# ALVI-Labs/frankenstein

Measured on AMD Instinct MI355X. Metric: neural frames/sec (train fwd+bwd+AdamW, whole job), higher is better.
Workload: dtype bf16; 1 GPU; brainformer-small (6L d=384 6x64 heads, N=6144 tokens) + 2-block perceiver, L1 head; fwd+bwd+clip+AdamW; per_gpu_batch=32, global_batch=32, frames_T=600, electrodes=256, parallelism=dp1, weights=random-init (seed 42)

## Files before the change

frankenstein_amd/csrc/gemm.hip:

```cpp
#include <type_traits>

#include "fk_common.h"

namespace {

#ifndef FK_EPI_UNROLL
#define FK_EPI_UNROLL 1
#endif
#include "gemm_tile.h"

struct NtArgs {
  const void* A; const void* B; void* C;
  const void* bias; const void* res;
  int64_t lda, ldb, ldc, ldr, res_rows;
  int M, N, K, vec_epi;
  int mode;
  void* aux; int64_t ldaux;
  const float* rope_table; int64_t rope_bs; int rope_T, rope_off, rope_D, rope_cols;
  int rope_qcols; int64_t rope_qoff;
};

#ifndef FK_NT_STORES_GEMM
#define FK_NT_STORES_GEMM 1
#endif
// ... 787 lines not shown
#pragma unroll
          for (int j = 0; j < 2; ++j) mma32<T>(acc[i][j], fb[j], fa[i]);
        __builtin_amdgcn_sched_barrier(0);
        if (s < 2) issue_b(fill_b, s); else issue_a(fill_a, s - 2);
        __builtin_amdgcn_sched_barrier(0);
      }
#else
      issue_b(fill_b, -1);
      issue_a(fill_a, -1);
#endif
      sa = sa == 2 ? 0 : sa + 1;
      sb ^= 1;
    }
    asm volatile("s_barrier" ::: "memory");
    char* stg = wave < 4 ? aslot(sa == 0 ? 2 : sa - 1) + wave * 8192 : bslot(sb ^ 1) + (wave - 4) * 8192;
#ifdef FK_RING_PROBE_NOEPI
    if (acc[0][0][0] == 123.456f) ((float*)p.C)[tid] = acc[MT - 1][1][3];
#else
#pragma unroll
    for (int i = 0; i < MT; ++i) {
      f32x16 (&sub)[1][2] = *reinterpret_cast<f32x16 (*)[1][2]>(&acc[i][0]);
      nt_epilogue<T, TO, true, 1, false, EPI>(p, sub, stg, m0 + wm * WM + i * 32, n0 + wn * 64, lane, false);
    }
#endif
  }
}

constexpr int R192_A = 256 * ROW_BYTES, R192_B = 192 * ROW_BYTES, R192_LDS = 3 * R192_A + 2 * R192_B + 8192;
static_assert(R192_LDS <= 160 * 1024, "LDS of a CU");

template <typename TO, int EPI>
__global__ __launch_bounds__(512, 2) void gemm_nt_ring192_kernel(NtArgs p) {
  using T = bf16_t;
  constexpr int BM_ = 256, BN_ = 192, APW = 4, BPW = 3, NT6 = 6;
  extern __shared__ __attribute__((aligned(16))) char smem[];
  auto aslot = [&](int i) -> char* { return smem + i * R192_A; };
  auto bslot = [&](int i) -> char* { return smem + 3 * R192_A + i * R192_B; };
  const int tid = threadIdx.x, lane = tid & 63;
  const int wave = __builtin_amdgcn_readfirstlane(tid >> 6);
  const int li = lane & 31, lh = lane >> 5;
  const int ntn = p.N / BN_;
  const TileRange tr = tile_range(((p.M + BM_ - 1) / BM_) * ntn);
  const int nbx = tr.nbx, t_end = tr.end;
  const int nk = p.K / 64;

  const T* srcA[APW];
  const T* srcB[BPW];
  auto set_a = [&](int tile) {
    const int m0 = (tile / ntn) * BM_;
#pragma unroll
    for (int j = 0; j < APW; ++j) srcA[j] = dma_src(p.A, m0, p.M, p.lda, wave * APW + j, lane);
  };
  auto set_b = [&](int tile) {
    const int n0 = (tile % ntn) * BN_;
#pragma unroll
    for (int j = 0; j < BPW; ++j) srcB[j] = dma_src<ROW_BYTES, false>(p.B, n0, p.N, p.ldb, wave * BPW + j, lane);
  };
  int atile = tr.beg + tr.jb, akt = 0, btile = atile, bkt = 0;
  if (atile < t_end) { set_a(atile); set_b(btile); }
  auto issue_a = [&](int slot, int part) __attribute__((always_inline)) {
    if (atile >= t_end) return;
    char* as = aslot(slot);
#pragma unroll
    for (int j = 0; j < APW; ++j)
      if (part < 0 || j / 2 == part)
        __builtin_amdgcn_global_load_lds((glb_void_t*)(srcA[j] + akt * 64), (lds_void_t*)(as + (wave * APW + j) * 1024), 16, 0, 0);
    if (part != 0) { if (++akt == nk) { akt = 0; atile += nbx; if (atile < t_end) set_a(atile); } }
  };
  auto issue_b = [&](int slot, int part) __attribute__((always_inline)) {
    if (btile >= t_end) return;
    char* bs = bslot(slot);
#pragma unroll
    for (int j = 0; j < BPW; ++j)
      if (part < 0 || (j + 1) / 2 == part)
        __builtin_amdgcn_global_load_lds((glb_void_t*)(srcB[j] + bkt * 64), (lds_void_t*)(bs + (wave * BPW + j) * 1024), 16, 0, 0);
    if (part != 0) { if (++bkt == nk) { bkt = 0; btile += nbx; if (btile < t_end) set_b(btile); } }
  };
  issue_a(0, -1);
  issue_b(0, -1);
  issue_a(1, -1);
  int sa = 0, sb = 0;
  for (int tile = tr.beg + tr.jb; tile < t_end; tile += nbx) {
    const int m0 = (tile / ntn) * BM_, n0 = (tile % ntn) * BN_;
    const bool last_tile = tile + nbx >= t_end;
    f32x16 acc[NT6];
#pragma unroll
    for (int j = 0; j < NT6; ++j)
#pragma unroll
      for (int r = 0; r < 16; ++r) acc[j][r] = 0.0f;
    for (int kt = 0; kt < nk; ++kt) {
      if (last_tile && kt == nk - 1) vm_wait_barrier<0>(); else vm_wait_barrier<APW>();
      const int fill_a = sa == 0 ? 2 : sa - 1, fill_b = sb ^ 1;
      const char* as = aslot(sa);
      const char* bs = bslot(sb);
#ifndef FK_RING_PROBE_NOMMA
#pragma unroll
      for (int s = 0; s < 4; ++s) {
        Frag<T> fa, fb[NT6];
        nt_frag<T>(fa, as, wave * 32 + li, s, lh);
#pragma unroll
        for (int j = 0; j < NT6; ++j) nt_frag<T>(fb[j], bs, j * 32 + li, s, lh);
#pragma unroll
        for (int j = 0; j < NT6; ++j) mma32<T>(acc[j], fb[j], fa);
        __builtin_amdgcn_sched_barrier(0);
        if (s < 2) issue_b(fill_b, s); else issue_a(fill_a, s - 2);
        __builtin_amdgcn_sched_barrier(0);
      }
#else
      issue_b(fill_b, -1);
      issue_a(fill_a, -1);
#endif
      sa = sa == 2 ? 0 : sa + 1;
      sb ^= 1;
    }
    asm volatile("s_barrier" ::: "memory");
    char* stg = wave < 4 ? aslot(sa == 0 ? 2 : sa - 1) + wave * 8192
              : (wave < 7 ? bslot(sb ^ 1) + (wave - 4) * 8192 : smem + 3 * R192_A + 2 * R192_B);
#ifdef FK_RING_PROBE_NOEPI
    if (acc[0][0] == 123.456f) ((float*)p.C)[tid] = acc[NT6 - 1][3];
#else
#pragma unroll
    for (int c = 0; c < 3; ++c) {
      f32x16 (&sub)[1][2] = *reinterpret_cast<f32x16 (*)[1][2]>(&acc[2 * c]);
      if (EPI == 0 && p.res) nt_epilogue<T, TO, true, 1, true, EPI>(p, sub, stg, m0 + wave * 32, n0 + 64 * c, lane, false);
      else nt_epilogue<T, TO, true, 1, false, EPI>(p, sub, stg, m0 + wave * 32, n0 + 64 * c, lane, false);
    }
#endif
  }
}

static unsigned persistent_grid(int64_t nt) {
  static const int g = [] { const char* e = getenv("FK_NT_GRID_MULT"); const int v = e ? atoi(e) : 4; return v < 1 ? 1 : (v > 64 ? 64 : v); }();
  const int64_t cap = 256LL * g;
  return (unsigned)(nt < cap ? nt : cap);
}

enum NtRoute { NT_RING2, NT_RING192, NT_RING128, NT_BIG, NT_GLDS4, NT_GLDS, NT_STAGED };

template <typename F> static void with_epi(const NtArgs& p, F f) {
  if (p.mode == 1) f(std::integral_constant<int, 1>{});
  else if (p.mode == 2) f(std::integral_constant<int, 2>{});
  else if (p.rope_table) f(std::integral_constant<int, 3>{});
  else f(std::integral_constant<int, 0>{});
}

template <typename TO> static void launch_nt_route(NtRoute route, const NtArgs& p, int64_t M, int64_t N, hipStream_t s) {
  const int64_t nwg = fk_cdiv(M, BM) * fk_cdiv(N, BN);
  const dim3 grid((unsigned)nwg), block(NTHREADS), block8(512);
  auto tiles256 = [&](int bn) { return dim3(persistent_grid(fk_cdiv(M, 256) * fk_cdiv(N, bn))); };
  switch (route) {
    case NT_RING2: {
      static const bool generic = getenv("FK_NT_RING2_GENERIC") != nullptr;
      if (generic) fk_launch_lds<gemm_nt_ring2_kernel<TO, -1>>(tiles256(256), block8, R2_LDS, s, p);
      else with_epi(p, [&](auto epi) { fk_launch_lds<gemm_nt_ring2_kernel<TO, decltype(epi)::value>>(tiles256(256), block8, R2_LDS, s, p); });
      break;
    }
    case NT_RING192: fk_launch_lds<gemm_nt_ring192_kernel<TO, 0>>(tiles256(192), block8, R192_LDS, s, p); break;
    case NT_RING128:
      with_epi(p, [&](auto epi) { fk_launch_lds<gemm_nt_ring_kernel<TO, 128, 128, 3, decltype(epi)::value>>(tiles256(128), block8, Ring<128, 128, 3>::LDS, s, p); });
      break;
    case NT_BIG: fk_launch_lds<gemm_nt_big_kernel<TO, 256>>(tiles256(256), block8, 2 * (256 + 256) * ROW_BYTES, s, p); break;
    case NT_GLDS4: fk_launch_lds<gemm_nt_glds4_kernel<TO>>(grid, block, G4_LDS, s, p); break;
    case NT_GLDS:
      hipLaunchKernelGGL((gemm_nt_glds_kernel<TO>), dim3((unsigned)(nwg < 512 ? nwg : 512)), block, 4 * TILE_BYTES, s, p);
      break;
    case NT_STAGED: hipLaunchKernelGGL((gemm_nt_kernel<bf16_t, TO>), grid, block, 4 * TILE_BYTES, s, p); break;
  }
}

template <typename T> struct TNT;
template <> struct TNT<bf16_t> { static constexpr int BKM = 64, ROWB = 256, CHUNKS = 16, STEPS = 4; };
template <> struct TNT<float> { static constexpr int BKM = 32, ROWB = 512, CHUNKS = 32, STEPS = 2; };

FK_DEV int tn_off_bf16(int row, int bytecol) {
  const int g = bytecol >> 6;
  return row * 256 + (((g ^ (row & 3)) << 6) | (bytecol & 63));
}

template <typename T> FK_DEV void tn_frag(Frag<T>& f, const char* tile, int cb, int s, int lane);
template <> FK_DEV void tn_frag<bf16_t>(Frag<bf16_t>& f, const char* tile, int cb, int s, int lane) {
  const int g = lane >> 4, i = lane & 15, h = g >> 1;
  const int col = cb + 16 * (g & 1) + 4 * (i & 3);
#pragma unroll
  for (int t = 0; t < 2; ++t) {
    const int row = 16 * s + 8 * h + 4 * t + (i >> 2);
    bf16x4 v = lds_read_tr4(reinterpret_cast<const bf16_t*>(tile + tn_off_bf16(row, col * 2)));
#pragma unroll
    for (int e = 0; e < 4; ++e) f.v[4 * t + e] = v[e];
  }
}
template <> FK_DEV void tn_frag<float>(Frag<float>& f, const char* tile, int cb, int s, int lane) {
  const int h = lane >> 5, c = cb + (lane & 31);
#pragma unroll
  for (int e = 0; e < 8; ++e)
    f.v[e] = *reinterpret_cast<const float*>(tile + (16 * s + 8 * h + e) * 512 + c * 4);
}

struct TnArgs {
  const void* A; const void* B; float* C; float* ws;
  int64_t lda, ldb, ldc;
  int M, N1, N2, rows_per_split, nsplit, accumulate;
};

template <typename T>
__global__ __launch_bounds__(NTHREADS, 2) void gemm_tn_kernel(TnArgs p) {
  extern __shared__ __attribute__((aligned(16))) char smem[];
  constexpr int BKM = TNT<T>::BKM, ROWB = TNT<T>::ROWB, CHUNKS = TNT<T>::CHUNKS, STEPS = TNT<T>::STEPS;
  constexpr int VEC = KT<T>::VEC;
  constexpr int LOG_CH = (CHUNKS == 16) ? 4 : 5;
  const int tid = threadIdx.x, lane = tid & 63, wave = tid >> 6;
  const int wm = wave >> 1, wn = wave & 1, li = lane & 31, lh = lane >> 5;
  const int nt2 = (p.N2 + BN - 1) / BN, ntiles = ((p.N1 + BM - 1) / BM) * nt2;
  const unsigned L = xcd_remap(blockIdx.x, gridDim.x);
  const int split = (int)(L / ntiles), tile = (int)(L % ntiles);
  const int a0 = (tile / nt2) * BM, b0 = (tile % nt2) * BN;
  const int mbeg = split * p.rows_per_split;
  const int mend = min(p.M, mbeg + p.rows_per_split);
  const T* A = (const T*)p.A;
  const T* B = (const T*)p.B;

  f32x16 acc[2][2];
#pragma unroll
  for (int i = 0; i < 2; ++i)
#pragma unroll
    for (int j = 0; j < 2; ++j)
#pragma unroll
      for (int r = 0; r < 16; ++r) acc[i][j][r] = 0.0f;

  u32x4 ra[4], rb[4];
  auto gload = [&](int mrow0) {
#pragma unroll
    for (int i = 0; i < 4; ++i) {
      const int id = tid + NTHREADS * i, row = id >> LOG_CH, ch = id & (CHUNKS - 1);
      const int m = mrow0 + row, ca = a0 + ch * VEC, cb = b0 + ch * VEC;
      u32x4 z = {0u, 0u, 0u, 0u};
      ra[i] = (m < mend && ca < p.N1) ? *reinterpret_cast<const u32x4*>(A + (int64_t)m * p.lda + ca) : z;
      rb[i] = (m < mend && cb < p.N2) ? *reinterpret_cast<const u32x4*>(B + (int64_t)m * p.ldb + cb) : z;
    }
  };
  auto lds_off = [&](int row, int ch) -> int {
    if constexpr (sizeof(T) == 2) return tn_off_bf16(row, ch * 16);
    else return row * ROWB + ch * 16;
  };
  auto lstore = [&](int buf) {
    char* as = smem + buf * 2 * TILE_BYTES;
    char* bs = as + TILE_BYTES;
#pragma unroll
    for (int i = 0; i < 4; ++i) {
      const int id = tid + NTHREADS * i, row = id >> LOG_CH, ch = id & (CHUNKS - 1);
      *reinterpret_cast<u32x4*>(as + lds_off(row, ch)) = ra[i];
      *reinterpret_cast<u32x4*>(bs + lds_off(row, ch)) = rb[i];
    }
  };

  const int nk = (mend - mbeg + BKM - 1) / BKM;
  if (nk > 0) {
    gload(mbeg);
    lstore(0);
  }
  __syncthreads();
  for (int kt = 0; kt < nk; ++kt) {
    if (kt + 1 < nk) gload(mbeg + (kt + 1) * BKM);
    const char* as = smem + (kt & 1) * 2 * TILE_BYTES;
    const char* bs = as + TILE_BYTES;
#pragma unroll
    for (int s = 0; s < STEPS; ++s) {
      Frag<T> fa[2], fb[2];
#pragma unroll
      for (int i = 0; i < 2; ++i) tn_frag<T>(fa[i], as, wm * 64 + i * 32, s, lane);
#pragma unroll
      for (int j = 0; j < 2; ++j) tn_frag<T>(fb[j], bs, wn * 64 + j * 32, s, lane);
#pragma unroll
      for (int i = 0; i < 2; ++i)
#pragma unroll
        for (int j = 0; j < 2; ++j) mma32<T>(acc[i][j], fa[i], fb[j]);
    }
    if (kt + 1 < nk) lstore((kt + 1) & 1);
    __syncthreads();
  }

  float* out = (p.nsplit > 1) ? p.ws + (int64_t)split * p.N1 * p.N2 : p.C;
  const int64_t ldo = (p.nsplit > 1) ? p.N2 : p.ldc;
  const bool accum = (p.nsplit == 1) && p.accumulate;
#pragma unroll
  for (int j = 0; j < 2; ++j) {
    const int n = b0 + wn * 64 + j * 32 + li;
    if (n >= p.N2) continue;
#pragma unroll
    for (int i = 0; i < 2; ++i)
#pragma unroll
      for (int r = 0; r < 16; ++r) {
        const int m = a0 + wm * 64 + i * 32 + acc_row(r, lh);
        if (m >= p.N1) continue;
        float* dst = out + (int64_t)m * ldo + n;
        *dst = accum ? (*dst + acc[i][j][r]) : acc[i][j][r];
      }
  }
}

constexpr int TG_A = 384, TG_B = 128, TG_K = 32;
#ifndef FK_TG_NS
#define FK_TG_NS 4
#endif
constexpr int TG_NS = FK_TG_NS;
constexpr int TG_A_ROW = TG_A * 2, TG_B_ROW = TG_B * 2;
constexpr int TG_A_BYTES = TG_K * TG_A_ROW, TG_B_BYTES = TG_K * TG_B_ROW, TG_STAGE = TG_A_BYTES + TG_B_BYTES;

template <int PITCH> FK_DEV int tg_off(int row, int bytecol) {
  return row * PITCH + (bytecol & ~255) + ((((bytecol >> 6) ^ row) & 3) << 6) + (bytecol & 63);
}
template <int OFF> FK_DEV bf16x4 tr_read(unsigned base) {
  s16x4 r;
  asm volatile("ds_read_b64_tr_b16 %0, %1 offset:%2" : "=v"(r) : "v"(base), "n"(OFF) : "memory");
  return __builtin_bit_cast(bf16x4, r);
}
template <int N> FK_DEV void lgkm_wait() {
  asm volatile("s_waitcnt lgkmcnt(%0)" ::"n"(N) : "memory");
  __builtin_amdgcn_sched_barrier(0);
}
template <int PITCH, int S> FK_DEV void tg_frag(Frag<bf16_t>& f, unsigned base) {
  const bf16x4 v0 = tr_read<(16 * S) * PITCH>(base), v1 = tr_read<(16 * S + 4) * PITCH>(base);
#pragma unroll
  for (int e = 0; e < 4; ++e) { f.v[e] = v0[e]; f.v[4 + e] = v1[e]; }
}
FK_DEV unsigned lds_addr(const char* p) {
  return (unsigned)(__UINTPTR_TYPE__)((__attribute__((address_space(3))) const char*)p);
}

template <int TB>
__global__ __launch_bounds__(512, 2) void gemm_tn_big_kernel(TnArgs p) {
  constexpr int B_ROW = TB == 128 ? 256 : 512, B_BYTES = TG_K * B_ROW, STAGE = TG_A_BYTES + B_BYTES, NJ = TB / 64, WB = TB / 2;
  using T = bf16_t;
  extern __shared__ __attribute__((aligned(16))) char smem[];
  const int tid = threadIdx.x, lane = tid & 63;
  const int wave = __builtin_amdgcn_readfirstlane(tid >> 6);
  const int wm = wave >> 1, wn = wave & 1, li = lane & 31, lh = lane >> 5;
  const int nt2 = p.N2 / TB, ntiles = (p.N1 / TG_A) * nt2;
  const unsigned L = xcd_remap(blockIdx.x, gridDim.x);
  const int split = (int)(L / ntiles), tile = (int)(L % ntiles);
  const int a0 = (tile / nt2) * TG_A, b0 = (tile % nt2) * TB;
  const int mbeg = split * p.rows_per_split;
  const int mend = min(p.M, mbeg + p.rows_per_split);
  const int nk = (mend - mbeg) / TG_K;

  constexpr int APW = TG_A_BYTES / 8192, BPW = B_BYTES / 8192, PER = APW + BPW;
  const T* srcA[APW];
  const T* srcB[BPW];
#pragma unroll
  for (int j = 0; j < APW; ++j) {
    const int o = (wave * APW + j) * 1024 + lane * 16, row = o / TG_A_ROW, bc = o % TG_A_ROW;
    const int sc = (bc & ~255) + ((((bc >> 6) ^ row) & 3) << 6) + (bc & 63);
    srcA[j] = (const T*)p.A + (int64_t)(mbeg + row) * p.lda + a0 + sc / 2;
  }
#pragma unroll
  for (int j = 0; j < BPW; ++j) {
    const int o = (wave * BPW + j) * 1024 + lane * 16, row = o / B_ROW, bc = o % B_ROW;
    int sc = (bc & ~255) + ((((bc >> 6) ^ row) & 3) << 6) + (bc & 63);
    if (sc >= TB * 2) sc = 0;
    srcB[j] = (const T*)p.B + (int64_t)(mbeg + row) * p.ldb + b0 + sc / 2;
  }
  const int64_t astep = (int64_t)TG_K * p.lda, bstep = (int64_t)TG_K * p.ldb;
  auto stage = [&](int buf) {
    char* as = smem + buf * STAGE;
#pragma unroll
    for (int j = 0; j < APW; ++j) {
      __builtin_amdgcn_global_load_lds((glb_void_t*)srcA[j], (lds_void_t*)(as + (wave * APW + j) * 1024), 16, 0, 0);
      srcA[j] += astep;
    }
#pragma unroll
    for (int j = 0; j < BPW; ++j) {
      __builtin_amdgcn_global_load_lds((glb_void_t*)srcB[j], (lds_void_t*)(as + TG_A_BYTES + (wave * BPW + j) * 1024), 16, 0, 0);
      srcB[j] += bstep;
    }
  };

  unsigned fbase[3 + NJ];
  {
    const int g = lane >> 4, i = lane & 15, row = 8 * (g >> 1) + (i >> 2), dc = 16 * (g & 1) + 4 * (i & 3);
#pragma unroll
    for (int q = 0; q < 3; ++q) fbase[q] = lds_addr(smem) + tg_off<TG_A_ROW>(row, (wm * 96 + q * 32 + dc) * 2);
#pragma unroll
    for (int q = 0; q < NJ; ++q) fbase[3 + q] = lds_addr(smem) + TG_A_BYTES + tg_off<B_ROW>(row, (wn * WB + q * 32 + dc) * 2);
  }

  f32x16 acc[3][NJ];
#pragma unroll
  for (int i = 0; i < 3; ++i)
#pragma unroll
    for (int j = 0; j < NJ; ++j)
#pragma unroll
      for (int r = 0; r < 16; ++r) acc[i][j][r] = 0.0f;

#pragma unroll
  for (int s = 0; s < TG_NS - 1; ++s)
    if (s < nk) stage(s);
  int slot = 0;
  for (int kt = 0; kt < nk; ++kt) {
    const int after = nk - 1 - kt;
    if (after >= TG_NS - 2) vm_wait_barrier<(TG_NS - 2) * PER>();
    else if (after == 3) vm_wait_barrier<3 * PER>();
    else if (after == 2) vm_wait_barrier<2 * PER>();
    else if (after == 1) vm_wait_barrier<PER>();
    else vm_wait_barrier<0>();
    if (kt + TG_NS - 1 < nk) stage(slot == 0 ? TG_NS - 1 : slot - 1);
    const unsigned bo = slot * STAGE;
    slot = slot == TG_NS - 1 ? 0 : slot + 1;
    Frag<T> f0[3 + NJ], f1[3 + NJ];
#pragma unroll
    for (int q = 0; q < 3; ++q) tg_frag<TG_A_ROW, 0>(f0[q], fbase[q] + bo);
#pragma unroll
    for (int q = 0; q < NJ; ++q) tg_frag<B_ROW, 0>(f0[3 + q], fbase[3 + q] + bo);
#pragma unroll
    for (int q = 0; q < 3; ++q) tg_frag<TG_A_ROW, 1>(f1[q], fbase[q] + bo);
#pragma unroll
    for (int q = 0; q < NJ; ++q) tg_frag<B_ROW, 1>(f1[3 + q], fbase[3 + q] + bo);
    lgkm_wait<2 * (3 + NJ)>();
#pragma unroll
    for (int i = 0; i < 3; ++i)
#pragma unroll
      for (int j = 0; j < NJ; ++j) mma32<T>(acc[i][j], f0[i], f0[3 + j]);
    lgkm_wait<0>();
#pragma unroll
    for (int i = 0; i < 3; ++i)
#pragma unroll
      for (int j = 0; j < NJ; ++j) mma32<T>(acc[i][j], f1[i], f1[3 + j]);
  }

  float* out = (p.nsplit > 1) ? p.ws + (int64_t)split * p.N1 * p.N2 : p.C;
  const int64_t ldo = (p.nsplit > 1) ? p.N2 : p.ldc;
  const bool accum = (p.nsplit == 1) && p.accumulate;
#pragma unroll
  for (int j = 0; j < NJ; ++j) {
    const int n = b0 + wn * WB + j * 32 + li;
#pragma unroll
    for (int i = 0; i < 3; ++i)
#pragma unroll
      for (int r = 0; r < 16; ++r) {
        const int m = a0 + wm * 96 + i * 32 + acc_row(r, lh);
        float* dst = out + (int64_t)m * ldo + n;
        *dst = accum ? (*dst + acc[i][j][r]) : acc[i][j][r];
      }
  }
}

__global__ __launch_bounds__(256) void reduce_slabs4_kernel(const float* ws, float* C, int64_t ldc, int N1, int N2, int nsplit, int accumulate) {
  const int64_t total = (int64_t)N1 * N2, total4 = total >> 2;
  const int n2v = N2 >> 2;
  for (int64_t i = blockIdx.x * (int64_t)blockDim.x + threadIdx.x; i < total4; i += (int64_t)gridDim.x * blockDim.x) {
    const f32x4* src = reinterpret_cast<const f32x4*>(ws) + i;
    f32x4 s = {0.0f, 0.0f, 0.0f, 0.0f};
    int k = 0;
    for (; k + 8 <= nsplit; k += 8) {
      f32x4 v[8];
#pragma unroll
      for (int u = 0; u < 8; ++u) v[u] = src[(int64_t)(k + u) * total4];
#pragma unroll
      for (int u = 0; u < 8; ++u) s += v[u];
    }
    for (; k < nsplit; ++k) s += src[(int64_t)k * total4];
    f32x4* dst = reinterpret_cast<f32x4*>(C + (i / n2v) * ldc + (i % n2v) * 4);
    if (accumulate) s += *dst;
    *dst = s;
  }
}
__global__ void reduce_slabs_kernel(const float* ws, float* C, int64_t ldc, int N1, int N2, int nsplit, int accumulate) {
  const int64_t total = (int64_t)N1 * N2;
  for (int64_t i = blockIdx.x * (int64_t)blockDim.x + threadIdx.x; i < total; i += (int64_t)gridDim.x * blockDim.x) {
    float s = 0.0f;
    for (int k = 0; k < nsplit; ++k) s += ws[k * total + i];
    float* dst = C + (i / N2) * ldc + (i % N2);
    *dst = accumulate ? (*dst + s) : s;
  }
}

template <typename T>
__global__ __launch_bounds__(256) void colsum_partial_kernel(const T* X, int64_t ld, float* part, int rows, int cols, int rows_per_blk) {
  constexpr int N = 16 / sizeof(T);
  __shared__ float red[256 * N];
  const int r0 = blockIdx.y * rows_per_blk, r1 = min(rows, r0 + rows_per_blk);
  const int cvt = (cols + N - 1) / N;
  {
    const int cv0 = blockIdx.x * 256;
    const int cvn = min(256, cvt - cv0), groups = 256 / cvn;
    const int vec = threadIdx.x % cvn, grp = threadIdx.x / cvn;
    float acc[N];
#pragma unroll
    for (int e = 0; e < N; ++e) acc[e] = 0.0f;
    if (grp < groups) {
      const T* p = X + (int64_t)(cv0 + vec) * N;
      for (int r = r0 + grp; r < r1; r += groups) {
        if constexpr (sizeof(T) == 2) {
          bf16x8 v = *reinterpret_cast<const bf16x8*>(p + (int64_t)r * ld);
#pragma unroll
          for (int e = 0; e < N; ++e) acc[e] += (float)v[e];
        } else {
          f32x4 v = *reinterpret_cast<const f32x4*>(p + (int64_t)r * ld);
#pragma unroll
          for (int e = 0; e < N; ++e) acc[e] += v[e];
        }
      }
    }
    __syncthreads();
#pragma unroll
    for (int e = 0; e < N; ++e) red[threadIdx.x * N + e] = acc[e];
    __syncthreads();
    if (threadIdx.x < cvn) {
#pragma unroll
      for (int e = 0; e < N; ++e) {
        float sm = 0.0f;
        for (int g2 = 0; g2 < groups; ++g2) sm += red[(g2 * cvn + threadIdx.x) * N + e];
        part[(int64_t)blockIdx.y * cols + (cv0 + threadIdx.x) * N + e] = sm;
      }
    }
  }
}
template <typename T>
__global__ void colsum_partial_scalar_kernel(const T* X, int64_t ld, float* part, int rows, int cols, int rows_per_blk) {
  const int c = blockIdx.x * blockDim.x + threadIdx.x;
  if (c >= cols) return;
  const int r0 = blockIdx.y * rows_per_blk, r1 = min(rows, r0 + rows_per_blk);
  float s = 0.0f;
  for (int r = r0; r < r1; ++r) s += to_f32<T>(X[(int64_t)r * ld + c]);
  part[(int64_t)blockIdx.y * cols + c] = s;
}
__global__ __launch_bounds__(256) void colsum_final_kernel(const float* part, float* out, int cols, int nblk, int accumulate) {
  __shared__ float red[256];
  const int c = blockIdx.x * 64 + (threadIdx.x & 63), g = threadIdx.x >> 6;
  float s = 0.0f;
  if (c < cols)
    for (int k = g; k < nblk; k += 4) s += part[(int64_t)k * cols + c];
  red[threadIdx.x] = s;
  __syncthreads();
  if (g == 0 && c < cols) {
    const float t = (red[threadIdx.x] + red[threadIdx.x + 64]) + (red[threadIdx.x + 128] + red[threadIdx.x + 192]);
    out[c] = accumulate ? out[c] + t : t;
  }
}

int tn_splits(int64_t M, int64_t N1, int64_t N2, int bkm) {
  const int64_t tiles = fk_cdiv(N1, BM) * fk_cdiv(N2, BN);
  int64_t want = fk_cdiv(1024, tiles);
  const int64_t maxs = fk_cdiv(M, (int64_t)bkm * 4);
  if (want >= 8) want = (want + 7) / 8 * 8;
  if (want > maxs) want = maxs;
  if (want < 1) want = 1;
  return (int)want;
}
bool tn_big_ok(int64_t M, int64_t N1, int64_t N2, int dtype) {
  return dtype == FK_BF16 && M % TG_K == 0 && M >= 16384 && N1 % TG_A == 0 && (N2 % TG_B == 0 || N2 % 192 == 0);
}
int tn_big_tb(int64_t N1, int64_t N2) {
  static const bool no192 = getenv("FK_TN_NO_192") != nullptr;
  if (N2 % TG_B != 0) return 192;
  return (N2 % 192 == 0 && N1 >= 2048 && !no192) ? 192 : TG_B;
}
int tn_big_splits(int64_t M, int64_t N1, int64_t N2) {
  const int64_t tiles = (N1 / TG_A) * (N2 / tn_big_tb(N1, N2));
  static const int mult = [] { const char* e = getenv("FK_TN_SPLIT_MULT"); const int v = e ? atoi(e) : 1; return v < 1 ? 1 : (v > 8 ? 8 : v); }();
  int64_t want = 256 / tiles * mult;
  const int64_t maxs = M / 512;
  if (want > maxs) want = maxs;
  if (want < 1) want = 1;
  return (int)want;
}
int colsum_blocks(int64_t rows) {
  int64_t b = fk_cdiv(rows, 256);
  if (b > 512) b = 512;
  if (b < 1) b = 1;
  return (int)b;
}

}

bool fk_qkv_rope_fused_ok(int64_t M, int64_t N, int64_t K, int64_t lda, int64_t ldb, int64_t ldc, const void* bias, int64_t T, int64_t D, int64_t rot_cols, int64_t q_cols, int dtype);
int fk_qkv_rope_fused_launch(const void* A, int64_t lda, const void* W, int64_t ldb, void* C, int64_t ldc, int64_t M, int64_t N, const float* table, int64_t table_bs, int64_t T, int64_t pos_off, int64_t rot_cols, int64_t q_cols, int64_t q_off, void* stream);
bool fk_mlp_up_fused_ok(int64_t M, int64_t H, int64_t K, int64_t lda, int64_t ldb, int64_t ldh, int64_t ldg, int dtype);
int fk_mlp_up_fused_launch(const void* A, int64_t lda, const void* W13, int64_t ldb, void* H13, int64_t ldh, void* G, int64_t ldg, int64_t M, int64_t H, void* stream);

extern "C" {

struct RopeSpec { const float* table; int64_t bs; int T, off, D, cols; int qcols; int64_t qoff; };

static int launch_nt(const char* name, const void* A, int64_t lda, const void* B, int64_t ldb, void* C, int64_t ldc, int64_t M,
                     int64_t N, int64_t K, const void* bias, const void* residual, int64_t ldr, int64_t res_rows, int dtype,
                     int out_dtype, int mode, void* aux, int64_t ldaux, void* stream, RopeSpec rope = RopeSpec{nullptr, 0, 1, 0, 2, 0, 0, 0}) {
  FK_CHECK_ARG(dtype == FK_F32 || dtype == FK_BF16, "%s: bad dtype %d", name, dtype);
  FK_CHECK_ARG(out_dtype == dtype || out_dtype == FK_F32, "%s: out_dtype must equal dtype or be f32", name);
  const int vec = dtype == FK_BF16 ? 8 : 4;
  FK_CHECK_ARG(M > 0 && N > 0 && K > 0, "%s: empty problem M=%lld N=%lld K=%lld", name, (long long)M, (long long)N, (long long)K);
  FK_CHECK_ARG(M < (1LL << 31) && N < (1LL << 31) && K < (1LL << 31), "%s: dims must fit int32", name);
  FK_CHECK_ARG(K % vec == 0 && lda % vec == 0 && ldb % vec == 0, "%s: K/lda/ldb must be multiples of %d", name, vec);
  const int64_t ccols = mode == 2 ? 2 * N : N, auxcols = mode == 1 ? N / 2 : (mode == 2 ? 2 * N : 0);
  FK_CHECK_ARG((M == 1 || (lda >= K && ldc >= ccols && ldaux >= auxcols && (!residual || res_rows == 1 || ldr >= N))) && (N == 1 || ldb >= K),
               "%s: leading dimensions must cover their rows (lda=%lld ldb=%lld K=%lld, ldc=%lld for %lld columns, aux %lld for %lld)", name,
               (long long)lda, (long long)ldb, (long long)K, (long long)ldc, (long long)ccols, (long long)ldaux, (long long)auxcols);
  FK_CHECK_ARG(A && B && C, "%s: null pointer", name);
  FK_CHECK_ARG(((uintptr_t)A & 15) == 0 && ((uintptr_t)B & 15) == 0, "%s: A/B must be 16-byte aligned", name);
  const int ovec = 8;
  const bool vec_epi = (N % ovec == 0) && (ldc % ovec == 0) && (((uintptr_t)C & 15) == 0) &&
                       (!residual || (ldr % ovec == 0 && ((uintptr_t)residual & 15) == 0));
  if (mode != 0)
    FK_CHECK_ARG(vec_epi && out_dtype == dtype && aux && ldaux % ovec == 0 && ((uintptr_t)aux & 15) == 0,
                 "%s: fused SwiGLU epilogue needs N %% 8 == 0 and 16-byte aligned, 8-element strided buffers", name);
  if (rope.table)
    FK_CHECK_ARG(vec_epi && rope.D % 8 == 0 && rope.cols % rope.D == 0 && rope.cols <= N && rope.T > 0 && M % rope.T == 0 &&
                 ((uintptr_t)rope.table & 15) == 0, "%s: fused RoPE needs the vector epilogue, D %% 8 == 0 and M %% T == 0", name);
  NtArgs p{A, B, C, bias, residual, lda, ldb, ldc, ldr, res_rows, (int)M, (int)N, (int)K, vec_epi ? 1 : 0, mode, aux, ldaux,
           rope.table, rope.bs, rope.T, rope.off, rope.D, rope.cols, rope.qcols, rope.qoff};
  const int64_t nwg = fk_cdiv(M, BM) * fk_cdiv(N, BN);
  hipStream_t s = (hipStream_t)stream;
  const bool glds = dtype == FK_BF16 && (K % 64 == 0);
  static const bool no_ring = getenv("FK_NT_NO_RING") != nullptr;
  const char* ring_min_env = getenv("FK_NT_RING_MIN_TILES");
  const int ring_min = ring_min_env ? atoi(ring_min_env) : 128;
  const bool wide = glds && M >= 4096 && vec_epi && !no_ring && fk_cdiv(M, 256) * fk_cdiv(N, 256) >= ring_min;
  const NtRoute route = [&] {
    if (wide && (N % 256 == 0 || (N % 128 == 0 && N >= 1024))) return NT_RING2;
    static const bool no_192 = getenv("FK_NT_NO_192") != nullptr;
    if (wide && N % 192 == 0 && N % 256 != 0 && N <= 768 && mode == 0 && !rope.table && !no_192) return NT_RING192;
    if (wide && N % 128 == 0) return NT_RING128;
    if (glds && M >= 4096 && N % 256 == 0 && vec_epi) return NT_BIG;
    static const bool no_g4 = getenv("FK_NT_NO_GLDS4") != nullptr;
    if (glds && nwg <= 256 && !no_g4) return NT_GLDS4;
    return glds ? NT_GLDS : NT_STAGED;
  }();
  if (dtype == FK_F32)
    hipLaunchKernelGGL((gemm_nt_kernel<float, float>), dim3((unsigned)nwg), dim3(NTHREADS), 4 * TILE_BYTES, s, p);
  else if (out_dtype == FK_BF16) launch_nt_route<bf16_t>(route, p, M, N, s);
  else launch_nt_route<float>(route, p, M, N, s);
  FK_CHECK_LAUNCH(name);
  return FK_OK;
}

int fk_gemm_nt(const void* A, int64_t lda, const void* B, int64_t ldb, void* C, int64_t ldc, int64_t M, int64_t N,
               int64_t K, const void* bias, const void* residual, int64_t ldr, int64_t res_rows, int dtype,
               int out_dtype, void* stream) {
  return launch_nt("fk_gemm_nt", A, lda, B, ldb, C, ldc, M, N, K, bias, residual, ldr, res_rows, dtype, out_dtype, 0, nullptr, 0, stream);
}

int fk_gemm_nt_rope(const void* A, int64_t lda, const void* B, int64_t ldb, void* C, int64_t ldc, int64_t M, int64_t N,
                    int64_t K, const void* bias, const float* table, int64_t table_bs, int64_t T, int64_t pos_off, int64_t D,
                    int64_t rot_cols, int64_t q_cols, int64_t q_table_off, int dtype, void* stream) {
  FK_CHECK_ARG(table && T > 0 && D > 0 && rot_cols >= 0, "fk_gemm_nt_rope: bad rope arguments");
  FK_CHECK_ARG(q_cols >= 0 && q_cols <= rot_cols && q_cols % 8 == 0 && q_table_off % 4 == 0, "fk_gemm_nt_rope: bad pre-scaled query table (q_cols %lld, offset %lld)", (long long)q_cols, (long long)q_table_off);
  if (A && B && C && (((uintptr_t)A | (uintptr_t)B | (uintptr_t)C | (uintptr_t)table) & 15) == 0 && M > 0 && pos_off >= 0 &&
      fk_qkv_rope_fused_ok(M, N, K, lda, ldb, ldc, bias, T, D, rot_cols, q_cols, dtype))
    return fk_qkv_rope_fused_launch(A, lda, B, ldb, C, ldc, M, N, table, table_bs, T, pos_off, rot_cols, q_cols, q_table_off, stream);
  return launch_nt("fk_gemm_nt_rope", A, lda, B, ldb, C, ldc, M, N, K, bias, nullptr, 0, 0, dtype, dtype, 0, nullptr, 0, stream,
                   RopeSpec{table, table_bs, (int)T, (int)pos_off, (int)D, (int)rot_cols, (int)q_cols, q_table_off});
}

int fk_gemm_nt_swiglu(const void* A, int64_t lda, const void* W13, int64_t ldb, void* H13, int64_t ldh, void* G,
                      int64_t ldg, int64_t M, int64_t H, int64_t K, int dtype, void* stream) {
  FK_CHECK_ARG(H > 0 && H % 4 == 0, "fk_gemm_nt_swiglu: hidden size must be a multiple of 4");
  if (A && W13 && H13 && G && (((uintptr_t)A | (uintptr_t)W13 | (uintptr_t)H13 | (uintptr_t)G) & 15) == 0 && M > 0 &&
      fk_mlp_up_fused_ok(M, H, K, lda, ldb, ldh, ldg, dtype))
    return fk_mlp_up_fused_launch(A, lda, W13, ldb, H13, ldh, G, ldg, M, H, stream);
  return launch_nt("fk_gemm_nt_swiglu", A, lda, W13, ldb, H13, ldh, M, 2 * H, K, nullptr, nullptr, 0, 0, dtype, dtype, 1, G, ldg, stream);
}

int fk_gemm_nt_dswiglu(const void* dY, int64_t lda, const void* W2T, int64_t ldb, const void* H13, int64_t ldh, void* dH13,
                       int64_t lddh, int64_t M, int64_t H, int64_t K, int dtype, void* stream) {
  FK_CHECK_ARG(H > 0 && H % 8 == 0, "fk_gemm_nt_dswiglu: hidden size must be a multiple of 8");
  FK_CHECK_ARG(lddh % 8 == 0 && ((uintptr_t)dH13 & 15) == 0, "fk_gemm_nt_dswiglu: dH13 must be 16-byte aligned with an 8-element stride");
  return launch_nt("fk_gemm_nt_dswiglu", dY, lda, W2T, ldb, dH13, lddh, M, H, K, nullptr, nullptr, 0, 0, dtype, dtype, 2,
                   const_cast<void*>(H13), ldh, stream);
}

size_t fk_gemm_tn_workspace_bytes(int64_t M, int64_t N1, int64_t N2, int dtype) {
  const int ns = tn_big_ok(M, N1, N2, dtype) ? tn_big_splits(M, N1, N2) : tn_splits(M, N1, N2, dtype == FK_BF16 ? 64 : 32);
  return ns > 1 ? (size_t)ns * N1 * N2 * sizeof(float) : 0;
}

int fk_gemm_tn(const void* A, int64_t lda, const void* B, int64_t ldb, float* C, int64_t ldc, int64_t M, int64_t N1,
               int64_t N2, int accumulate, int dtype, void* workspace, size_t workspace_bytes, void* stream) {
  FK_CHECK_ARG(dtype == FK_F32 || dtype == FK_BF16, "fk_gemm_tn: bad dtype %d", dtype);
  const int vec = dtype == FK_BF16 ? 8 : 4, bkm = dtype == FK_BF16 ? 64 : 32;
  FK_CHECK_ARG(M > 0 && N1 > 0 && N2 > 0, "fk_gemm_tn: empty problem");
  FK_CHECK_ARG(M < (1LL << 31) && N1 < (1LL << 31) && N2 < (1LL << 31), "fk_gemm_tn: dims must fit int32");
  FK_CHECK_ARG(N1 % vec == 0 && N2 % vec == 0 && lda % vec == 0 && ldb % vec == 0,
               "fk_gemm_tn: N1/N2/lda/ldb must be multiples of %d (N1=%lld N2=%lld)", vec, (long long)N1, (long long)N2);
  FK_CHECK_ARG(((uintptr_t)A & 15) == 0 && ((uintptr_t)B & 15) == 0, "fk_gemm_tn: A/B must be 16-byte aligned");
  const bool big = tn_big_ok(M, N1, N2, dtype);
  const int ns = big ? tn_big_splits(M, N1, N2) : tn_splits(M, N1, N2, bkm);
  const size_t need = ns > 1 ? (size_t)ns * N1 * N2 * sizeof(float) : 0;
  FK_CHECK_ARG(workspace_bytes >= need && (need == 0 || workspace), "fk_gemm_tn: workspace too small (%zu < %zu)", workspace_bytes, need);
  int64_t rps = fk_cdiv(fk_cdiv(M, ns), bkm) * bkm;
  TnArgs p{A, B, C, (float*)workspace, lda, ldb, ldc, (int)M, (int)N1, (int)N2, (int)rps, ns, accumulate};
  dim3 grid((unsigned)(fk_cdiv(N1, BM) * fk_cdiv(N2, BN) * ns)), block(NTHREADS);
  hipStream_t s = (hipStream_t)stream;
  if (big) {
    const int tb = tn_big_tb(N1, N2);
    dim3 bgrid((unsigned)((N1 / TG_A) * (N2 / tb) * ns));
    if (tb == 192) {
      constexpr int LDS192 = TG_NS * (TG_A_BYTES + TG_K * 512);
      fk_launch_lds<gemm_tn_big_kernel<192>>(bgrid, dim3(512), LDS192, s, p);
    } else {
      fk_launch_lds<gemm_tn_big_kernel<128>>(bgrid, dim3(512), TG_NS * TG_STAGE, s, p);
    }
  } else if (dtype == FK_BF16) hipLaunchKernelGGL((gemm_tn_kernel<bf16_t>), grid, block, 4 * TILE_BYTES, s, p);
  else hipLaunchKernelGGL((gemm_tn_kernel<float>), grid, block, 4 * TILE_BYTES, s, p);
  FK_CHECK_LAUNCH("fk_gemm_tn");
  if (ns > 1) {
    const int64_t total = N1 * N2;
    if (N2 % 4 == 0 && ldc % 4 == 0 && (((uintptr_t)C | (uintptr_t)workspace) & 15) == 0) {
      int nb = (int)fk_cdiv(total / 4, 256);
      if (nb > 2048) nb = 2048;
      hipLaunchKernelGGL(reduce_slabs4_kernel, dim3(nb), dim3(256), 0, s, (const float*)workspace, C, ldc, (int)N1, (int)N2, ns, accumulate);
    } else {
      int nb = (int)fk_cdiv(total, 256);
      if (nb > 2048) nb = 2048;
      hipLaunchKernelGGL(reduce_slabs_kernel, dim3(nb), dim3(256), 0, s, (const float*)workspace, C, ldc, (int)N1, (int)N2, ns, accumulate);
    }
    FK_CHECK_LAUNCH("fk_gemm_tn(reduce)");
  }
  return FK_OK;
}

size_t fk_colsum_workspace_bytes(int64_t rows, int64_t cols) { return (size_t)colsum_blocks(rows) * cols * sizeof(float); }

int fk_colsum(const void* X, int64_t ld, float* out, int64_t rows, int64_t cols, int accumulate, int dtype,
              void* workspace, size_t workspace_bytes, void* stream) {
  FK_CHECK_ARG(dtype == FK_F32 || dtype == FK_BF16, "fk_colsum: bad dtype %d", dtype);
  FK_CHECK_ARG(rows > 0 && cols > 0 && rows < (1LL << 31) && cols < (1LL << 31), "fk_colsum: bad shape");
  const int nb = colsum_blocks(rows);
  FK_CHECK_ARG(workspace && workspace_bytes >= (size_t)nb * cols * sizeof(float), "fk_colsum: workspace too small");
  const int rpb = (int)fk_cdiv(rows, nb);
  hipStream_t s = (hipStream_t)stream;
  const int vec = dtype == FK_BF16 ? 8 : 4;
  if (cols % vec == 0 && ld % vec == 0 && ((uintptr_t)X & 15) == 0) {
    dim3 grid((unsigned)fk_cdiv(fk_cdiv(cols, vec), 256), (unsigned)nb), block(256);
    if (dtype == FK_BF16) hipLaunchKernelGGL(colsum_partial_kernel<bf16_t>, grid, block, 0, s, (const bf16_t*)X, ld, (float*)workspace, (int)rows, (int)cols, rpb);
    else hipLaunchKernelGGL(colsum_partial_kernel<float>, grid, block, 0, s, (const float*)X, ld, (float*)workspace, (int)rows, (int)cols, rpb);
  } else {
    dim3 grid((unsigned)fk_cdiv(cols, 256), (unsigned)nb), block(256);
    if (dtype == FK_BF16) hipLaunchKernelGGL(colsum_partial_scalar_kernel<bf16_t>, grid, block, 0, s, (const bf16_t*)X, ld, (float*)workspace, (int)rows, (int)cols, rpb);
    else hipLaunchKernelGGL(colsum_partial_scalar_kernel<float>, grid, block, 0, s, (const float*)X, ld, (float*)workspace, (int)rows, (int)cols, rpb);
  }
  FK_CHECK_LAUNCH("fk_colsum(partial)");
  hipLaunchKernelGGL(colsum_final_kernel, dim3((unsigned)fk_cdiv(cols, 64)), dim3(256), 0, s, (const float*)workspace, out, (int)cols, nb, accumulate);
  FK_CHECK_LAUNCH("fk_colsum(final)");
  return FK_OK;
}

}
```

Measured before the change: 399,200 frames/s.

## Use 16x16x32 MFMA path in big TN weight-grad GEMM with extra LDS swizzle

```diff
diff --git a/frankenstein_amd/csrc/gemm.hip b/frankenstein_amd/csrc/gemm.hip
--- a/frankenstein_amd/csrc/gemm.hip
+++ b/frankenstein_amd/csrc/gemm.hip
@@ -1113,19 +1113,22 @@
 #ifndef FK_TG_NS
 #define FK_TG_NS 4
 #endif
+#ifndef FK_TN_M16
+#define FK_TN_M16 2
+#endif
 constexpr int TG_NS = FK_TG_NS;
 constexpr int TG_A_ROW = TG_A * 2, TG_B_ROW = TG_B * 2;
 constexpr int TG_A_BYTES = TG_K * TG_A_ROW, TG_B_BYTES = TG_K * TG_B_ROW, TG_STAGE = TG_A_BYTES + TG_B_BYTES;
 
-template <int PITCH> FK_DEV int tg_off(int row, int bytecol) {
-  return row * PITCH + (bytecol & ~255) + ((((bytecol >> 6) ^ row) & 3) << 6) + (bytecol & 63);
-}
+FK_DEV int tg_swz(int row, int bc) { return (bc & ~255) + ((((bc >> 6) ^ row) & 3) << 6) + ((bc & 63) ^ ((row & 8) << 2)); }
+template <int PITCH> FK_DEV int tg_off(int row, int bytecol) { return row * PITCH + tg_swz(row, bytecol); }
 template <int OFF> FK_DEV bf16x4 tr_read(unsigned base) {
   s16x4 r;
   asm volatile("ds_read_b64_tr_b16 %0, %1 offset:%2" : "=v"(r) : "v"(base), "n"(OFF) : "memory");
   return __builtin_bit_cast(bf16x4, r);
 }
 template <int N> FK_DEV void lgkm_wait() {
+  __builtin_amdgcn_sched_barrier(0);
   asm volatile("s_waitcnt lgkmcnt(%0)" ::"n"(N) : "memory");
   __builtin_amdgcn_sched_barrier(0);
 }
@@ -1140,6 +1143,7 @@
 
 template <int TB>
 __global__ __launch_bounds__(512, 2) void gemm_tn_big_kernel(TnArgs p) {
+  constexpr bool M16 = (FK_TN_M16 >> (TB == 192 ? 1 : 0)) & 1;
   constexpr int B_ROW = TB == 128 ? 256 : 512, B_BYTES = TG_K * B_ROW, STAGE = TG_A_BYTES + B_BYTES, NJ = TB / 64, WB = TB / 2;
   using T = bf16_t;
   extern __shared__ __attribute__((aligned(16))) char smem[];
@@ -1160,13 +1164,13 @@
 #pragma unroll
   for (int j = 0; j < APW; ++j) {
     const int o = (wave * APW + j) * 1024 + lane * 16, row = o / TG_A_ROW, bc = o % TG_A_ROW;
-    const int sc = (bc & ~255) + ((((bc >> 6) ^ row) & 3) << 6) + (bc & 63);
+    const int sc = tg_swz(row, bc);
     srcA[j] = (const T*)p.A + (int64_t)(mbeg + row) * p.lda + a0 + sc / 2;
   }
 #pragma unroll
   for (int j = 0; j < BPW; ++j) {
     const int o = (wave * BPW + j) * 1024 + lane * 16, row = o / B_ROW, bc = o % B_ROW;
-    int sc = (bc & ~255) + ((((bc >> 6) ^ row) & 3) << 6) + (bc & 63);
+    int sc = tg_swz(row, bc);
     if (sc >= TB * 2) sc = 0;
     srcB[j] = (const T*)p.B + (int64_t)(mbeg + row) * p.ldb + b0 + sc / 2;
   }
@@ -1185,72 +1189,125 @@
     }
   };
 
-  unsigned fbase[3 + NJ];
-  {
-    const int g = lane >> 4, i = lane & 15, row = 8 * (g >> 1) + (i >> 2), dc = 16 * (g & 1) + 4 * (i & 3);
-#pragma unroll
-    for (int q = 0; q < 3; ++q) fbase[q] = lds_addr(smem) + tg_off<TG_A_ROW>(row, (wm * 96 + q * 32 + dc) * 2);
-#pragma unroll
-    for (int q = 0; q < NJ; ++q) fbase[3 + q] = lds_addr(smem) + TG_A_BYTES + tg_off<B_ROW>(row, (wn * WB + q * 32 + dc) * 2);
-  }
-
-  f32x16 acc[3][NJ];
-#pragma unroll
-  for (int i = 0; i < 3; ++i)
-#pragma unroll
-    for (int j = 0; j < NJ; ++j)
-#pragma unroll
-      for (int r = 0; r < 16; ++r) acc[i][j][r] = 0.0f;
-
-#pragma unroll
-  for (int s = 0; s < TG_NS - 1; ++s)
-    if (s < nk) stage(s);
-  int slot = 0;
-  for (int kt = 0; kt < nk; ++kt) {
-    const int after = nk - 1 - kt;
-    if (after >= TG_NS - 2) vm_wait_barrier<(TG_NS - 2) * PER>();
-    else if (after == 3) vm_wait_barrier<3 * PER>();
-    else if (after == 2) vm_wait_barrier<2 * PER>();
-    else if (after == 1) vm_wait_barrier<PER>();
-    else vm_wait_barrier<0>();
-    if (kt + TG_NS - 1 < nk) stage(slot == 0 ? TG_NS - 1 : slot - 1);
-    const unsigned bo = slot * STAGE;
-    slot = slot == TG_NS - 1 ? 0 : slot + 1;
-    Frag<T> f0[3 + NJ], f1[3 + NJ];
-#pragma unroll
-    for (int q = 0; q < 3; ++q) tg_frag<TG_A_ROW, 0>(f0[q], fbase[q] + bo);
-#pragma unroll
-    for (int q = 0; q < NJ; ++q) tg_frag<B_ROW, 0>(f0[3 + q], fbase[3 + q] + bo);
-#pragma unroll
-    for (int q = 0; q < 3; ++q) tg_frag<TG_A_ROW, 1>(f1[q], fbase[q] + bo);
-#pragma unroll
-    for (int q = 0; q < NJ; ++q) tg_frag<B_ROW, 1>(f1[3 + q], fbase[3 + q] + bo);
-    lgkm_wait<2 * (3 + NJ)>();
-#pragma unroll
-    for (int i = 0; i < 3; ++i)
-#pragma unroll
-      for (int j = 0; j < NJ; ++j) mma32<T>(acc[i][j], f0[i], f0[3 + j]);
-    lgkm_wait<0>();
-#pragma unroll
-    for (int i = 0; i < 3; ++i)
-#pragma unroll
-      for (int j = 0; j < NJ; ++j) mma32<T>(acc[i][j], f1[i], f1[3 + j]);
-  }
-
   float* out = (p.nsplit > 1) ? p.ws + (int64_t)split * p.N1 * p.N2 : p.C;
   const int64_t ldo = (p.nsplit > 1) ? p.N2 : p.ldc;
   const bool accum = (p.nsplit == 1) && p.accumulate;
-#pragma unroll
-  for (int j = 0; j < NJ; ++j) {
-    const int n = b0 + wn * WB + j * 32 + li;
+
+  auto ring = [&](auto&& compute) {
+#pragma unroll
+    for (int s = 0; s < TG_NS - 1; ++s)
+      if (s < nk) stage(s);
+    int slot = 0;
+    for (int kt = 0; kt < nk; ++kt) {
+      const int after = nk - 1 - kt;
+      if (after >= TG_NS - 2) vm_wait_barrier<(TG_NS - 2) * PER>();
+      else if (after == 3) vm_wait_barrier<3 * PER>();
+      else if (after == 2) vm_wait_barrier<2 * PER>();
+      else if (after == 1) vm_wait_barrier<PER>();
+      else vm_wait_barrier<0>();
+      if (kt + TG_NS - 1 < nk) stage(slot == 0 ? TG_NS - 1 : slot - 1);
+      const unsigned bo = slot * STAGE;
+      slot = slot == TG_NS - 1 ? 0 : slot + 1;
+      compute(bo);
+    }
+  };
+
+  if constexpr (M16) {
+    constexpr int NA = 6, NB = TB / 32;
+    unsigned fbase[NA + NB];
+    {
+      const int g = lane >> 4, i = lane & 15, row = 8 * g + (i >> 2), dc = 4 * (i & 3);
+#pragma unroll
+      for (int q = 0; q < NA; ++q) fbase[q] = lds_addr(smem) + tg_off<TG_A_ROW>(row, (wm * 96 + q * 16 + dc) * 2);
+#pragma unroll
+      for (int q = 0; q < NB; ++q) fbase[NA + q] = lds_addr(smem) + TG_A_BYTES + tg_off<B_ROW>(row, (wn * WB + q * 16 + dc) * 2);
+    }
+    f32x4 acc[NA][NB];
+#pragma unroll
+    for (int i = 0; i < NA; ++i)
+#pragma unroll
+      for (int j = 0; j < NB; ++j) acc[i][j] = f32x4{0.0f, 0.0f, 0.0f, 0.0f};
+
+    ring([&](unsigned bo) {
+      Frag<T> fa[NA], fb[NB];
+#pragma unroll
+      for (int q = 0; q < NA / 2; ++q) tg_frag<TG_A_ROW, 0>(fa[q], fbase[q] + bo);
+#pragma unroll
+      for (int q = 0; q < NB; ++q) tg_frag<B_ROW, 0>(fb[q], fbase[NA + q] + bo);
+#pragma unroll
+      for (int q = NA / 2; q < NA; ++q) tg_frag<TG_A_ROW, 0>(fa[q], fbase[q] + bo);
+      lgkm_wait<NA>();
+#pragma unroll
+      for (int i = 0; i < NA / 2; ++i)
+#pragma unroll
+        for (int j = 0; j < NB; ++j) acc[i][j] = __builtin_amdgcn_mfma_f32_16x16x32_bf16(fa[i].v, fb[j].v, acc[i][j], 0, 0, 0);
+      lgkm_wait<0>();
+#pragma unroll
+      for (int i = NA / 2; i < NA; ++i)
+#pragma unroll
+        for (int j = 0; j < NB; ++j) acc[i][j] = __builtin_amdgcn_mfma_f32_16x16x32_bf16(fa[i].v, fb[j].v, acc[i][j], 0, 0, 0);
+    });
+
+#pragma unroll
+    for (int i = 0; i < NA; ++i)
+#pragma unroll
+      for (int r = 0; r < 4; ++r) {
+        const int m = a0 + wm * 96 + i * 16 + 4 * (lane >> 4) + r;
+        float* dst = out + (int64_t)m * ldo + b0 + wn * WB + (lane & 15);
+#pragma unroll
+        for (int j = 0; j < NB; ++j) dst[j * 16] = accum ? (dst[j * 16] + acc[i][j][r]) : acc[i][j][r];
+      }
+  } else {
+    unsigned fbase[3 + NJ];
+    {
+      const int g = lane >> 4, i = lane & 15, row = 8 * (g >> 1) + (i >> 2), dc = 16 * (g & 1) + 4 * (i & 3);
+#pragma unroll
+      for (int q = 0; q < 3; ++q) fbase[q] = lds_addr(smem) + tg_off<TG_A_ROW>(row, (wm * 96 + q * 32 + dc) * 2);
+#pragma unroll
+      for (int q = 0; q < NJ; ++q) fbase[3 + q] = lds_addr(smem) + TG_A_BYTES + tg_off<B_ROW>(row, (wn * WB + q * 32 + dc) * 2);
+    }
+    f32x16 acc[3][NJ];
 #pragma unroll
     for (int i = 0; i < 3; ++i)
 #pragma unroll
-      for (int r = 0; r < 16; ++r) {
-        const int m = a0 + wm * 96 + i * 32 + acc_row(r, lh);
-        float* dst = out + (int64_t)m * ldo + n;
-        *dst = accum ? (*dst + acc[i][j][r]) : acc[i][j][r];
-      }
+      for (int j = 0; j < NJ; ++j)
+#pragma unroll
+        for (int r = 0; r < 16; ++r) acc[i][j][r] = 0.0f;
+
+    ring([&](unsigned bo) {
+      Frag<T> f0[3 + NJ], f1[3 + NJ];
+#pragma unroll
+      for (int q = 0; q < 3; ++q) tg_frag<TG_A_ROW, 0>(f0[q], fbase[q] + bo);
+#pragma unroll
+      for (int q = 0; q < NJ; ++q) tg_frag<B_ROW, 0>(f0[3 + q], fbase[3 + q] + bo);
+#pragma unroll
+      for (int q = 0; q < 3; ++q) tg_frag<TG_A_ROW, 1>(f1[q], fbase[q] + bo);
+#pragma unroll
+      for (int q = 0; q < NJ; ++q) tg_frag<B_ROW, 1>(f1[3 + q], fbase[3 + q] + bo);
+      lgkm_wait<2 * (3 + NJ)>();
+#pragma unroll
+      for (int i = 0; i < 3; ++i)
+#pragma unroll
+        for (int j = 0; j < NJ; ++j) mma32<T>(acc[i][j], f0[i], f0[3 + j]);
+      lgkm_wait<0>();
+#pragma unroll
+      for (int i = 0; i < 3; ++i)
+#pragma unroll
+        for (int j = 0; j < NJ; ++j) mma32<T>(acc[i][j], f1[i], f1[3 + j]);
+    });
+
+#pragma unroll
+    for (int j = 0; j < NJ; ++j) {
+      const int n = b0 + wn * WB + j * 32 + li;
+#pragma unroll
+      for (int i = 0; i < 3; ++i)
+#pragma unroll
+        for (int r = 0; r < 16; ++r) {
+          const int m = a0 + wm * 96 + i * 32 + acc_row(r, lh);
+          float* dst = out + (int64_t)m * ldo + n;
+          *dst = accum ? (*dst + acc[i][j][r]) : acc[i][j][r];
+        }
+    }
   }
 }
 
@@ -1363,7 +1420,7 @@
 int tn_big_tb(int64_t N1, int64_t N2) {
   static const bool no192 = getenv("FK_TN_NO_192") != nullptr;
   if (N2 % TG_B != 0) return 192;
-  return (N2 % 192 == 0 && N1 >= 2048 && !no192) ? 192 : TG_B;
+  return (N2 % 192 == 0 && (N1 / TG_A) * (N2 / 192) >= 6 && !no192) ? 192 : TG_B;
 }
 int tn_big_splits(int64_t M, int64_t N1, int64_t N2) {
   const int64_t tiles = (N1 / TG_A) * (N2 / tn_big_tb(N1, N2));
@@ -1503,12 +1560,9 @@
   if (big) {
     const int tb = tn_big_tb(N1, N2);
     dim3 bgrid((unsigned)((N1 / TG_A) * (N2 / tb) * ns));
-    if (tb == 192) {
-      constexpr int LDS192 = TG_NS * (TG_A_BYTES + TG_K * 512);
-      fk_launch_lds<gemm_tn_big_kernel<192>>(bgrid, dim3(512), LDS192, s, p);
-    } else {
-      fk_launch_lds<gemm_tn_big_kernel<128>>(bgrid, dim3(512), TG_NS * TG_STAGE, s, p);
-    }
+    constexpr int LDS192 = TG_NS * (TG_A_BYTES + TG_K * 512);
+    if (tb == 192) fk_launch_lds<gemm_tn_big_kernel<192>>(bgrid, dim3(512), LDS192, s, p);
+    else fk_launch_lds<gemm_tn_big_kernel<128>>(bgrid, dim3(512), TG_NS * TG_STAGE, s, p);
   } else if (dtype == FK_BF16) hipLaunchKernelGGL((gemm_tn_kernel<bf16_t>), grid, block, 4 * TILE_BYTES, s, p);
   else hipLaunchKernelGGL((gemm_tn_kernel<float>), grid, block, 4 * TILE_BYTES, s, p);
   FK_CHECK_LAUNCH("fk_gemm_tn");
```

New measurement: 401,400 frames/s, median of 6. Within noise of the previous version (+0.6%).
